# slackhq/nebula

Measured on AMD Instinct MI355X. Metric: GiB/s device-resident AES-256-GCM seal+open, 1300 B pkts, 64 Ki batch, higher is better.
Workload: dtype u8; 1 GPU; C2 AES-256-GCM, 1 tunnel key, 65536 x 1300 B packets, device-resident; packets_per_gpu=65536, payload_bytes_per_pkt=1300, keys=1, cipher=AES-256-GCM, parallelism=1 GPU(s), independent packet shards, no collective

## Files before the change

### nebula_amd/csrc/aes_gcm.hip

```cpp
#include <hip/hip_runtime.h>

#include <atomic>
#include <hip/hip_ext.h>

#include <cstdlib>
#include <cstring>
#include <stdint.h>

#include <type_traits>

#include "../../include/nebula_aead.h"
#include "device_common.hpp"
#include "knobs.hpp"
#include "layout.hpp"
#include "rxwin.hpp"
#include "sched.hpp"
#include "timing.hpp"

#ifdef NEB_ISA_MARKS
#define NEB_MARK(x) asm volatile(";NEBMARK " #x)
#else
#define NEB_MARK(x) ((void)0)
#endif

namespace neb {


struct T0Table {
    uint32_t t[256];
};
constexpr uint8_t kSbox[256] = {
    0x63,0x7c,0x77,0x7b,0xf2,0x6b,0x6f,0xc5,0x30,0x01,0x67,0x2b,0xfe,0xd7,0xab,0x76,
    0xca,0x82,0xc9,0x7d,0xfa,0x59,0x47,0xf0,0xad,0xd4,0xa2,0xaf,0x9c,0xa4,0x72,0xc0,
    0xb7,0xfd,0x93,0x26,0x36,0x3f,0xf7,0xcc,0x34,0xa5,0xe5,0xf1,0x71,0xd8,0x31,0x15,
    0x04,0xc7,0x23,0xc3,0x18,0x96,0x05,0x9a,0x07,0x12,0x80,0xe2,0xeb,0x27,0xb2,0x75,
    0x09,0x83,0x2c,0x1a,0x1b,0x6e,0x5a,0xa0,0x52,0x3b,0xd6,0xb3,0x29,0xe3,0x2f,0x84,
    0x53,0xd1,0x00,0xed,0x20,0xfc,0xb1,0x5b,0x6a,0xcb,0xbe,0x39,0x4a,0x4c,0x58,0xcf,
    0xd0,0xef,0xaa,0xfb,0x43,0x4d,0x33,0x85,0x45,0xf9,0x02,0x7f,0x50,0x3c,0x9f,0xa8,
    0x51,0xa3,0x40,0x8f,0x92,0x9d,0x38,0xf5,0xbc,0xb6,0xda,0x21,0x10,0xff,0xf3,0xd2,
    0xcd,0x0c,0x13,0xec,0x5f,0x97,0x44,0x17,0xc4,0xa7,0x7e,0x3d,0x64,0x5d,0x19,0x73,
    0x60,0x81,0x4f,0xdc,0x22,0x2a,0x90,0x88,0x46,0xee,0xb8,0x14,0xde,0x5e,0x0b,0xdb,
    0xe0,0x32,0x3a,0x0a,0x49,0x06,0x24,0x5c,0xc2,0xd3,0xac,0x62,0x91,0x95,0xe4,0x79,
    0xe7,0xc8,0x37,0x6d,0x8d,0xd5,0x4e,0xa9,0x6c,0x56,0xf4,0xea,0x65,0x7a,0xae,0x08,
    0xba,0x78,0x25,0x2e,0x1c,0xa6,0xb4,0xc6,0xe8,0xdd,0x74,0x1f,0x4b,0xbd,0x8b,0x8a,
    0x70,0x3e,0xb5,0x66,0x48,0x03,0xf6,0x0e,0x61,0x35,0x57,0xb9,0x86,0xc1,0x1d,0x9e,
    0xe1,0xf8,0x98,0x11,0x69,0xd9,0x8e,0x94,0x9b,0x1e,0x87,0xe9,0xce,0x55,0x28,0xdf,
    0x8c,0xa1,0x89,0x0d,0xbf,0xe6,0x42,0x68,0x41,0x99,0x2d,0x0f,0xb0,0x54,0xbb,0x16};

constexpr uint8_t xt(uint8_t a) { return (uint8_t)((a << 1) ^ ((a & 0x80) ? 0x1b : 0)); }
constexpr T0Table make_t0() {
    T0Table r{};
    for (int i = 0; i < 256; i++) {
        uint32_t s = kSbox[i], s2 = xt(kSbox[i]), s3 = s2 ^ s;
        r.t[i] = s2 | (s << 8) | (s << 16) | (s3 << 24);
    }
    return r;
}
__constant__ T0Table c_T0 = make_t0();


__device__ __forceinline__ uint32_t x3(uint32_t a, uint32_t b, uint32_t c) {
    uint32_t r;
    asm("v_bitop3_b32 %0, %1, %2, %3 bitop3:0x96" : "=v"(r) : "v"(a), "v"(b), "v"(c));
    return r;
}
__device__ __forceinline__ uint32_t x3s(uint32_t a, uint32_t b, uint32_t k) {
    uint32_t r;
    asm("v_bitop3_b32 %0, %1, %2, %3 bitop3:0x96" : "=v"(r) : "v"(a), "v"(b), "s"(k));
    return r;
}
__device__ __forceinline__ uint32_t rotl8(uint32_t x) { return __builtin_amdgcn_alignbit(x, x, 24); }
__device__ __forceinline__ uint4 xor4(uint4 a, uint4 b) { return make_uint4(a.x ^ b.x, a.y ^ b.y, a.z ^ b.z, a.w ^ b.w); }
__device__ __forceinline__ uint4 x34(uint4 a, uint4 b, uint4 c) {
    return make_uint4(x3(a.x, b.x, c.x), x3(a.y, b.y, c.y), x3(a.z, b.z, c.z), x3(a.w, b.w, c.w));
}
__device__ __forceinline__ uint4 sel4(bool c, uint4 a, uint4 b) {
    return make_uint4(c ? a.x : b.x, c ? a.y : b.y, c ? a.z : b.z, c ? a.w : b.w);
}
__device__ __forceinline__ uint4 bswap4(uint4 v) { return make_uint4(bswap32(v.x), bswap32(v.y), bswap32(v.z), bswap32(v.w)); }
__device__ __forceinline__ uint4 shfl_xor4(uint4 v, int m) {
    return make_uint4(__shfl_xor(v.x, m), __shfl_xor(v.y, m), __shfl_xor(v.z, m), __shfl_xor(v.w, m));
}
__device__ __forceinline__ uint32_t byte_of(uint32_t w, int k) {
    return k == 0 ? (w & 0xFFu) : (k == 3 ? (w >> 24) : __builtin_amdgcn_ubfe(w, 8 * k, 8));
}

template <class T>
__device__ __forceinline__ T lds_at(const void* base, uint32_t byte_off) {
    return *reinterpret_cast<const T*>(
        __builtin_assume_aligned(reinterpret_cast<const char*>(base) + byte_off, sizeof(T)));
}

__device__ __forceinline__ uint2 ttab_lane_base(uint32_t lane, uint32_t high = 0u) {
    const uint32_t c = lane & 31u, hi = c >> 4;
    return make_uint2((c << 3) | (hi << 2) | high, (c << 3) | ((hi ^ 1u) << 2) | high);
}
__device__ __forceinline__ uint2 ttab_entry(uint32_t i) {
    const uint32_t t = c_T0.t[i >> 5], t2 = __builtin_amdgcn_alignbit(t, t, 16);
    return (i & 16u) ? make_uint2(t2, t) : make_uint2(t, t2);
}

#ifndef NEB_PRIO
#define NEB_PRIO 3
#endif
#ifndef NEB_PRIO_AGE
#define NEB_PRIO_AGE 1
#endif

struct RkRegs {
    const uint32_t* k;
    static constexpr bool kUniform = true;
    static constexpr int kPrioHi = NEB_PRIO, kPrioLo = 0;
    __device__ __forceinline__ uint4 get(int r) const {
        return make_uint4(k[4 * r], k[4 * r + 1], k[4 * r + 2], k[4 * r + 3]);
    }
};
template <int HI, int LO>
struct RkRegsPrio : RkRegs {
    static constexpr int kPrioHi = HI, kPrioLo = LO;
};
struct RkLds {
    const uint4* base;
    static constexpr bool kUniform = false;
    static constexpr int kPrioHi = NEB_PRIO, kPrioLo = 0;
    __device__ __forceinline__ uint4 get(int r) const { return base[r]; }
};

struct TLook {
    const uint2* ttab;
    uint2 lb;
    __device__ __forceinline__ uint32_t t0(uint32_t s, int k) const {
        return lds_at<uint32_t>(ttab, perm(s, lb.x, 0x0C020000u | ((4u + (uint32_t)k) << 8)));
    }
    __device__ __forceinline__ uint32_t t2(uint32_t s, int k) const {
        return lds_at<uint32_t>(ttab, perm(s, lb.y, 0x0C020000u | ((4u + (uint32_t)k) << 8)));
    }
    __device__ __forceinline__ uint32_t t1(uint32_t s, int k) const { return rotl8(t0(s, k)); }
    __device__ __forceinline__ uint32_t t3(uint32_t s, int k) const { return rotl8(t2(s, k)); }
    __device__ __forceinline__ uint32_t t1r(uint32_t s, int k) const { return t0(s, k); }
    __device__ __forceinline__ uint32_t t3r(uint32_t s, int k) const { return t2(s, k); }
    static constexpr bool kFour = false;
};

__device__ __forceinline__ uint32_t ttab4_lane_base(uint32_t lane) {
    const uint32_t c = lane & 31u, hi = c >> 4;
    return ((c << 3) | (hi << 2)) | (1u << 16) | (((c << 3) | ((hi ^ 1u) << 2)) << 24);
}
__device__ __forceinline__ uint2 ttab4_entry(uint32_t i) {
    uint32_t t = c_T0.t[(i >> 5) & 255u];
    if (i & 8192u) t = __builtin_amdgcn_alignbit(t, t, 16);
    const uint32_t t1 = rotl8(t);
    return (i & 16u) ? make_uint2(t1, t) : make_uint2(t, t1);
}
template <uint32_t N, uint32_t THREADS, class F>
__device__ __forceinline__ void fill_ttab(uint2* dst, uint32_t tid, F entry) {
    constexpr uint32_t K = (N + THREADS - 1) / THREADS;
    constexpr bool kWhole = N % THREADS == 0;
    uint2 v[K];
#pragma unroll
    for (uint32_t j = 0; j < K; j++) v[j] = entry((tid + j * THREADS) % N);
#pragma unroll
    for (uint32_t j = 0; j < K; j++)
        if (kWhole || tid + j * THREADS < N) dst[tid + j * THREADS] = v[j];
}
struct TLook4 {
    const uint2* ttab;
    uint32_t lb;
    __device__ __forceinline__ uint32_t at(uint32_t s, int k, uint32_t sel) const {
        return lds_at<uint32_t>(ttab, perm(s, lb, sel | ((4u + (uint32_t)k) << 8)));
    }
    __device__ __forceinline__ uint32_t t0(uint32_t s, int k) const { return at(s, k, 0x0C0C0000u); }
    __device__ __forceinline__ uint32_t t1(uint32_t s, int k) const { return at(s, k, 0x0C0C0003u); }
    __device__ __forceinline__ uint32_t t2(uint32_t s, int k) const { return at(s, k, 0x0C020000u); }
// ... 134 lines not shown
    const uint32_t u1 = c.L.y ^ T.t3(t0, 3);
    const uint32_t u2 = c.L.z ^ T.t2(t0, 2);
    const uint32_t u3 = c.L.w ^ T.t1(t0, 1);
    return aes256_rounds<3>(u0, u1, u2, u3, T, rk);
}


__device__ __forceinline__ uint4 gf_mulx(uint4 v) {
    uint32_t lsb = v.w & 1u;
    uint4 r;
    r.w = shr64(v.z, v.w, 1);
    r.z = shr64(v.y, v.z, 1);
    r.y = shr64(v.x, v.y, 1);
    r.x = (v.x >> 1) ^ (lsb ? 0xE1000000u : 0u);
    return r;
}

__device__ __forceinline__ uint4 gf_reduce(const uint32_t z[8]) {
    const uint32_t l0 = z[4], l1 = z[5], l2 = z[6], l3 = z[7];
    uint32_t t0 = x3(l0, l0 >> 1, l0 >> 2) ^ (l0 >> 7);
    uint32_t t1 = x3(x3(l1, shr64(l0, l1, 1), shr64(l0, l1, 2)), shr64(l0, l1, 7), z[1]);
    uint32_t t2 = x3(x3(l2, shr64(l1, l2, 1), shr64(l1, l2, 2)), shr64(l1, l2, 7), z[2]);
    uint32_t t3 = x3(x3(l3, shr64(l2, l3, 1), shr64(l2, l3, 2)), shr64(l2, l3, 7), z[3]);
    uint32_t o = x3(l3 << 31, l3 << 30, l3 << 25);
    uint32_t of = x3(o, o >> 1, o >> 2) ^ (o >> 7);
    return make_uint4(x3(z[0], t0, of), t1, t2, t3);
}

__device__ __forceinline__ uint4 gf_mul_xpow(uint4 q, uint32_t i) {
    const uint32_t w = i >> 5, b = i & 31u;
    const uint32_t src[4] = {q.x, q.y, q.z, q.w};
    uint32_t y[8], z[8];
#pragma unroll
    for (int k = 0; k < 8; k++) {
        uint32_t v = 0;
#pragma unroll
        for (int j = 0; j < 4; j++) v = (uint32_t)(k - j) == w ? src[j] : v;
        y[k] = v;
    }
    z[0] = y[0] >> b;
#pragma unroll
    for (int k = 1; k < 8; k++) z[k] = shr64(y[k - 1], y[k], b);
    return gf_reduce(z);
}

__device__ __forceinline__ uint4 gf_mul_xpow32(uint4 q, uint32_t b) {
    const uint32_t z[8] = {q.x >> b, shr64(q.x, q.y, b), shr64(q.y, q.z, b), shr64(q.z, q.w, b), shr64(q.w, 0u, b),
                           0u, 0u, 0u};
    return gf_reduce(z);
}

template <int K>
__device__ __forceinline__ uint32_t byte_hi_nibble(uint32_t w) {
    uint32_t r;
    if constexpr (K == 0) {
        r = w & 0xF0u;
    } else {
        asm("v_and_b32_sdwa %0, %1, %2 dst_sel:DWORD dst_unused:UNUSED_PAD src0_sel:BYTE_%c3 src1_sel:DWORD"
            : "=v"(r) : "v"(w), "s"(0xF0u), "i"(K));
    }
    return r;
}

__device__ __forceinline__ uint4 gf_mul_full(uint4 x, uint4 acc, const uint4* ftab) {
    const uint32_t xw[4] = {x.x, x.y, x.z, x.w};
#pragma unroll
    for (int q = 0; q < 4; q++) {
        const uint32_t hi = xw[q];
        const uint32_t lo = xw[q] << 4;
        const uint32_t ah[4] = {byte_hi_nibble<0>(hi), byte_hi_nibble<1>(hi), byte_hi_nibble<2>(hi),
                                byte_hi_nibble<3>(hi)};
        const uint32_t al[4] = {byte_hi_nibble<0>(lo), byte_hi_nibble<1>(lo), byte_hi_nibble<2>(lo),
                                byte_hi_nibble<3>(lo)};
#pragma unroll
        for (int k = 0; k < 4; k++) {
            const uint4 e1 = lds_at<uint4>(ftab, (uint32_t)(8 * q + 6 - 2 * k) * 256u + ah[k]);
            const uint4 e2 = lds_at<uint4>(ftab, (uint32_t)(8 * q + 7 - 2 * k) * 256u + al[k]);
            acc = x34(acc, e1, e2);
        }
    }
    return acc;
}

__device__ __forceinline__ uint4 gf_mul_pos(uint4 x, const uint4* ptab) {
    const uint32_t xw[4] = {x.x, x.y, x.z, x.w};
    uint32_t z[8] = {0, 0, 0, 0, 0, 0, 0, 0};
#pragma unroll
    for (int q = 0; q < 4; q++) {
        const uint32_t hi = xw[q], lo = xw[q] << 4;
        const uint32_t ah[4] = {byte_hi_nibble<0>(hi), byte_hi_nibble<1>(hi), byte_hi_nibble<2>(hi),
                                byte_hi_nibble<3>(hi)};
        const uint32_t al[4] = {byte_hi_nibble<0>(lo), byte_hi_nibble<1>(lo), byte_hi_nibble<2>(lo),
                                byte_hi_nibble<3>(lo)};
#pragma unroll
        for (int k = 0; k < 4; k++) {
            const uint4 e1 = lds_at<uint4>(ptab, (uint32_t)(6 - 2 * k) * 256u + ah[k]);
            const uint4 e2 = lds_at<uint4>(ptab, (uint32_t)(7 - 2 * k) * 256u + al[k]);
            z[q] = x3(z[q], e1.x, e2.x);
            z[q + 1] = x3(z[q + 1], e1.y, e2.y);
            z[q + 2] = x3(z[q + 2], e1.z, e2.z);
            z[q + 3] = x3(z[q + 3], e1.w, e2.w);
        }
    }
    return gf_reduce(z);
}

__device__ __forceinline__ void gf_acc_pos(uint4 x, const uint4* ptab, uint32_t z[8]) {
    const uint32_t xw[4] = {x.x, x.y, x.z, x.w};
#pragma unroll
    for (int q = 0; q < 4; q++) {
        const uint32_t hi = xw[q], lo = xw[q] << 4;
        const uint32_t ah[4] = {byte_hi_nibble<0>(hi), byte_hi_nibble<1>(hi), byte_hi_nibble<2>(hi),
                                byte_hi_nibble<3>(hi)};
        const uint32_t al[4] = {byte_hi_nibble<0>(lo), byte_hi_nibble<1>(lo), byte_hi_nibble<2>(lo),
                                byte_hi_nibble<3>(lo)};
#pragma unroll
        for (int k = 0; k < 4; k++) {
            const uint4 e1 = lds_at<uint4>(ptab, (uint32_t)(6 - 2 * k) * 256u + ah[k]);
            const uint4 e2 = lds_at<uint4>(ptab, (uint32_t)(7 - 2 * k) * 256u + al[k]);
            z[q] = x3(z[q], e1.x, e2.x);
            z[q + 1] = x3(z[q + 1], e1.y, e2.y);
            z[q + 2] = x3(z[q + 2], e1.z, e2.z);
            z[q + 3] = x3(z[q + 3], e1.w, e2.w);
        }
    }
}

__device__ __forceinline__ uint4 gf_mul_pos_off(uint4 x, const void* base, uint32_t off) {
    const uint32_t xw[4] = {x.x, x.y, x.z, x.w};
    uint32_t z[8] = {0, 0, 0, 0, 0, 0, 0, 0};
#pragma unroll
    for (int q = 0; q < 4; q++) {
        const uint32_t hi = xw[q], lo = xw[q] << 4;
        const uint32_t ah[4] = {byte_hi_nibble<0>(hi), byte_hi_nibble<1>(hi), byte_hi_nibble<2>(hi),
                                byte_hi_nibble<3>(hi)};
        const uint32_t al[4] = {byte_hi_nibble<0>(lo), byte_hi_nibble<1>(lo), byte_hi_nibble<2>(lo),
                                byte_hi_nibble<3>(lo)};
#pragma unroll
        for (int k = 0; k < 4; k++) {
            const uint4 e1 = lds_at<uint4>(base, (uint32_t)(6 - 2 * k) * 256u + (ah[k] | off));
            const uint4 e2 = lds_at<uint4>(base, (uint32_t)(7 - 2 * k) * 256u + (al[k] | off));
            z[q] = x3(z[q], e1.x, e2.x);
            z[q + 1] = x3(z[q + 1], e1.y, e2.y);
            z[q + 2] = x3(z[q + 2], e1.z, e2.z);
            z[q + 3] = x3(z[q + 3], e1.w, e2.w);
        }
    }
    return gf_reduce(z);
}

__device__ __forceinline__ uint4 gf_mul_shoup(uint4 x, uint32_t tab, const uint4* base) {
    const uint32_t xw[4] = {x.x, x.y, x.z, x.w};
    uint32_t hi[4], lo[4];
#pragma unroll
    for (int q = 0; q < 4; q++) {
        hi[q] = xw[q] & 0xF0F0F0F0u;
        lo[q] = (xw[q] << 4) & 0xF0F0F0F0u;
    }
    uint32_t z[8] = {0, 0, 0, 0, 0, 0, 0, 0};
#pragma unroll
    for (int r = 0; r < 8; r++) {
        const int k = 3 - (r >> 1);
        uint4 m[4];
#pragma unroll
        for (int q = 0; q < 4; q++) {
            const uint32_t src = (r & 1) ? lo[q] : hi[q];
// ... 120 lines not shown
        const uint64_t abits = (uint64_t)d.aad_len * 8u, cbits = (uint64_t)d.len * 8u;
        X = make_uint4((uint32_t)(abits >> 32), (uint32_t)abits, (uint32_t)(cbits >> 32), (uint32_t)cbits);
        ej0.set(ks);
    }
    return X;
}

template <int CM, class TL, class RK>
__device__ __forceinline__ uint4 gcm_lane_ks(const LaneBlock& b, uint32_t c1, uint32_t c2, const CtrConst& cc,
                                             const TL& T, const RK& rk) {
    if constexpr (CM == 2) return aes256_ctr8_block(cc, b.ctr, T, rk);
    else if constexpr (CM == 1) return aes256_ctr_block(cc, b.ctr, T, rk);
    else return aes256_block(0u, c1, c2, bswap32(b.ctr), T, rk);
}

template <bool OPEN>
__device__ __forceinline__ uint32_t gcm_finish(const neb_desc& d, uint4 S, uint4 ej0, uint32_t lane, uint32_t l,
                                               uint32_t LPP, uint8_t* arena) {
    const uint4 tag = xor4(ej0, bswap4(S));
    uint32_t fail = 0;
    if (l == LPP - 1u) {
        if constexpr (!OPEN) {
            store_block(arena + d.dst_off + d.len, tag, 16);
        } else {
            const uint4 rt = load_block(arena + d.src_off + d.len, 16);
            const uint4 df = xor4(rt, tag);
            fail = (df.x | df.y | df.z | df.w) != 0u;
        }
    }
    if constexpr (OPEN) {
        fail = (uint32_t)__shfl((int)fail, (int)(lane | (LPP - 1u)));
        if (fail) {
            for (uint32_t off = 16u * l; off < d.len; off += 16u * LPP)
                store_block(arena + d.dst_off + off, make_uint4(0, 0, 0, 0), min(16u, d.len - off));
        }
    }
    return fail;
}


constexpr uint32_t kLg = 2;
constexpr uint32_t kLpp = 1u << kLg;
constexpr uint32_t kPpw = 64u / kLpp;
static_assert(kLpp == kFullPow, "the single-key Horner stride is the full table's power");

__device__ __forceinline__ uint4 shfl4(uint4 v, uint32_t src) {
    return make_uint4(__shfl(v.x, (int)src), __shfl(v.y, (int)src), __shfl(v.z, (int)src), __shfl(v.w, (int)src));
}
__device__ __forceinline__ uint4 shfl_down4(uint4 v, uint32_t d) {
    return make_uint4(__shfl_down(v.x, d), __shfl_down(v.y, d), __shfl_down(v.z, d), __shfl_down(v.w, d));
}

struct FinalPermLanes {
    uint32_t src1, src2, off;
};
__device__ __forceinline__ FinalPermLanes final_perm_lanes(uint32_t lane, const uint32_t tab_off[4]) {
    const uint32_t c = (lane >> 2) & 7u, h = lane >> 5;
    const uint32_t g = ((uint32_t)__popc(c) & 1u) + 2u * h;
    const uint32_t i = 4u * (c >> 1) + (lane & 3u);
    const uint32_t l = lane & 3u, q = lane >> 2, m = q >> 2;
    const uint32_t b = (l & 1u) ^ ((uint32_t)__popc(m) & 1u);
    FinalPermLanes f;
    f.src1 = 4u * i + g;
    f.src2 = 32u * (l >> 1) + 4u * (2u * m + b) + (q & 3u);
    f.off = g == 0u ? tab_off[0] : g == 1u ? tab_off[1] : g == 2u ? tab_off[2] : tab_off[3];
    return f;
}
template <int CTRL>
__device__ __forceinline__ uint4 dpp4(uint4 v) {
    return make_uint4((uint32_t)__builtin_amdgcn_mov_dpp((int)v.x, CTRL, 0xF, 0xF, false),
                      (uint32_t)__builtin_amdgcn_mov_dpp((int)v.y, CTRL, 0xF, 0xF, false),
                      (uint32_t)__builtin_amdgcn_mov_dpp((int)v.z, CTRL, 0xF, 0xF, false),
                      (uint32_t)__builtin_amdgcn_mov_dpp((int)v.w, CTRL, 0xF, 0xF, false));
}
template <class MUL>
__device__ __forceinline__ uint4 final_perm(uint4 A, const FinalPermLanes& fp, MUL&& mul) {
    const uint4 a = shfl4(A, fp.src1);
    uint4 v = shfl4(mul(a, fp.off), fp.src2);
    v = xor4(v, dpp4<0xB1>(v));
    return xor4(v, dpp4<0x4E>(v));
}

struct GhFullPerm {
    const uint4* full;
    const void* base;
    FinalPermLanes fp;
    __device__ __forceinline__ uint4 horner(uint4 a, uint32_t) const {
        return gf_mul_full(a, make_uint4(0, 0, 0, 0), full);
    }
    __device__ __forceinline__ uint4 final(uint4 A, uint32_t, uint32_t) const {
        return final_perm(A, fp, [&](uint4 a, uint32_t off) { return gf_mul_pos_off(a, base, off); });
    }
};

template <class OFF>
__device__ __forceinline__ uint4 tree_final(uint4 A, uint32_t lane, uint32_t lg, const uint4* base, OFF&& shoup_off) {
    uint4 V = A;
    for (uint32_t i = 0; i < lg; i++) V = xor4(gf_mul_shoup(V, shoup_off(i), base), shfl_down4(V, 1u << i));
    V = gf_mul_shoup(V, shoup_off(0u), base);
    return shfl4(V, lane & ~((1u << lg) - 1u));
}

#ifndef NEB_TAIL_TREE
#define NEB_TAIL_TREE 0
#endif
struct GhShoup64 {
    const uint4* m16;
    const uint4* shoup;
    const uint4* pos;
    const uint4* hi;
    __device__ __forceinline__ uint4 horner(uint4 a, uint32_t) const { return gf_mul_pos(a, pos); }
    __device__ __forceinline__ uint4 final(uint4 A, uint32_t lane, uint32_t lg) const {
#if NEB_TAIL_TREE
        return tree_final(A, lane, lg, shoup, [](uint32_t i) { return i * 256u; });
#else
        const uint32_t b = lane & 15u, a = (lane >> 4) & 3u;
        uint4 V = gf_mul_shoup(A, (15u - b) * 256u, m16);
        V = xor4(V, shfl_xor4(V, 8));
        V = xor4(V, shfl_xor4(V, 4));
        V = xor4(V, shfl_xor4(V, 2));
        V = xor4(V, shfl_xor4(V, 1));
        const uint4 W = gf_mul_shoup(V, (a < 3u ? 2u - a : 0u) * 256u, hi);
        V = a < 3u ? W : V;
        V = xor4(V, shfl_xor4(V, 16));
        return xor4(V, shfl_xor4(V, 32));
#endif
    }
};

struct GhChunk4 {
    const uint4* shoup;
    const uint4* pos;
    __device__ __forceinline__ uint4 horner(uint4 a, uint32_t) const { return gf_mul_pos(a, pos); }
    __device__ __forceinline__ uint4 final(uint4 A, uint32_t lane, uint32_t) const {
        const uint32_t ln = lane;
        const uint32_t tab_off[4] = {3u * 256u, 2u * 256u, 256u, 0u};
        return final_perm(A, final_perm_lanes(ln, tab_off),
                          [&](uint4 a, uint32_t off) { return gf_mul_shoup(a, off, shoup); });
    }
};
struct GhChunkTail {
    const uint4* shoup;
    const uint4* pos;
    __device__ __forceinline__ uint4 horner(uint4 a, uint32_t) const { return gf_mul_pos(a, pos); }
    __device__ __forceinline__ uint4 final(uint4 A, uint32_t lane, uint32_t lg) const {
        const uint32_t ln = lane;
        const uint32_t tab_off[4] = {3u * 256u, 2u * 256u, 256u, 0u};
        const uint4 Q = final_perm(A, final_perm_lanes(ln, tab_off),
                                   [&](uint4 a, uint32_t off) { return gf_mul_shoup(a, off, shoup); });
        const uint32_t a = (ln >> 2) & ((1u << (lg - 2u)) - 1u);
        const uint4 W = sel4((a & 1u) != 0u, Q, gf_mul_shoup(Q, 3u * 256u, shoup));
        const uint4 P = xor4(W, shfl_xor4(W, 4));
        if (lg == 3u) return P;
        const uint4 U = sel4((a & 2u) != 0u, P, gf_mul_shoup(P, 4u * 256u, shoup));
        return xor4(U, shfl_xor4(U, 8));
    }
};

constexpr uint32_t kCsHdrMask = 0xFFFu;
__device__ __forceinline__ uint32_t le16_sum(uint4 v) {
    return (v.x & 0xFFFFu) + (v.x >> 16) + (v.y & 0xFFFFu) + (v.y >> 16) + (v.z & 0xFFFFu) + (v.z >> 16) +
           (v.w & 0xFFFFu) + (v.w >> 16);
}
__device__ __forceinline__ uint32_t block_byte(uint4 v, uint32_t q) {
    const uint32_t w = q < 4u ? v.x : q < 8u ? v.y : q < 12u ? v.z : v.w;
    return (w >> (8u * (q & 3u))) & 0xFFu;
}
__device__ __forceinline__ uint32_t cs_fold16(uint32_t s) {
    s = (s & 0xFFFFu) + (s >> 16);
    s = (s & 0xFFFFu) + (s >> 16);
    return s;
// ... 126 lines not shown
        auto horner = [&](uint32_t r) -> uint4 { return r == 0 ? make_uint4(0, 0, 0, 0) : gh.horner(A, lg); };
        auto tround = [&](uint32_t r) {
            NEB_MARK(round_begin);
            if (r < sh.R) {
                const LaneBlock b = lane_block(sh, r, l, lg);
                const bool fast = fast_round(b);
                uint4 pre = make_uint4(0, 0, 0, 0);
                if (fast) pre = fast_load(b);
                const uint4 G = horner(r);
                __builtin_amdgcn_sched_barrier(0);
                uint4 ks = make_uint4(0, 0, 0, 0);
                if (__any(b.is_ct || b.is_len)) ks = gcm_lane_ks<CM>(b, c1, c2, cc, T, rk);
                io(b, G, ks, fast, pre);
            }
            NEB_MARK(round_end);
        };
        for (uint32_t r = 0; __any(r < sh.R); r++) tround(r);
    };
#if NEB_ONE_TRACE
    const uint64_t tp0 = __builtin_amdgcn_s_memrealtime();
#endif
    if (__all(sh.m + 1u < 256u)) rounds(std::integral_constant<int, 2>{});
    else if (__all(sh.m + 1u < 65536u)) rounds(std::integral_constant<int, 1>{});
    else rounds(std::integral_constant<int, 0>{});
    if constexpr (CS) {
        for (uint32_t sft = 1; sft < LPP; sft <<= 1) {
            cs_acc += (uint32_t)__shfl_xor((int)cs_acc, (int)sft);
            cs_fk |= (uint32_t)__shfl_xor((int)cs_fk, (int)sft);
        }
    }
#if NEB_ONE_TRACE
    __builtin_amdgcn_s_waitcnt(0);
    const uint64_t tp1 = __builtin_amdgcn_s_memrealtime();
#endif
#ifdef NEB_WAVE_TRACE
    const uint64_t tq2 = phase_now();
    phase_add(1, tq1, tq2);
#endif
    NEB_MARK(rounds_done);
    uint4 V = gh.final(A, lane, lg);
    NEB_MARK(final_done);
#ifdef NEB_WAVE_TRACE
    const uint64_t tq3 = phase_now();
    phase_add(2, tq2, tq3);
#endif
#if NEB_ONE_TRACE
    __builtin_amdgcn_s_waitcnt(0);
    const uint64_t tp2 = __builtin_amdgcn_s_memrealtime();
    if (lane == 0) printf("  rounds %u  final %u (x10 ns, R=%u)\n", (unsigned)(tp1 - tp0), (unsigned)(tp2 - tp1), sh.R);
#endif
    if constexpr (CS) {
        if (run && cs_on && l == LPP - 1u) V = xor4(V, gcm_csum_fix(d, sh.n, sh.na, cs_acc, cs_fk, args.arena, cs_pow));
    }
    if (run && gcm_finish<OPEN>(d, V, ej0.get(), lane, l, LPP, args.arena)) st = NEB_STATUS_AUTH_FAILED;
    if (valid && l == LPP - 1u) args.status[p] = (int32_t)st;
    NEB_MARK(grp_end);
#ifdef NEB_WAVE_TRACE
    phase_add(3, tq3, phase_now());
#endif
}

__device__ __forceinline__ void load_round_keys(const uint32_t* rec, uint32_t rks[60]) {
#pragma unroll
    for (int i = 0; i < 60; i++) rks[i] = __builtin_amdgcn_readfirstlane(rec[kRecRoundKeys + i]);
}

#ifdef NEB_WAVE_TRACE
constexpr uint32_t kWaveTraceSlots = 64, kWaveTraceWaves = 8192, kWaveTraceCap = kWaveTraceSlots * kWaveTraceWaves;
__device__ uint4 g_wtrace[kWaveTraceCap];
__device__ __forceinline__ void wave_trace(uint32_t lane, uint32_t slot, uint32_t a, uint32_t b, uint64_t t0,
                                           uint64_t t1) {
    const uint32_t w = blockIdx.x * (blockDim.x >> 6) + (threadIdx.x >> 6);
    if (lane == 0u && w < kWaveTraceWaves && slot < kWaveTraceSlots)
        g_wtrace[w * kWaveTraceSlots + slot] = make_uint4(a | 0x80000000u, b, (uint32_t)t0, (uint32_t)t1);
}
#endif


constexpr int kSingleWaves = 16;
constexpr int kSingleWpe = 4;
constexpr int kSingleThreads = kSingleWaves * kWave;

struct SingleLds {
    uint4 full[32 * 16];
    uint4 pos1[8 * 16];
    uint2 ttab[2 * 256 * 32];
    uint4 pos23[2][8 * 16];
};
struct SingleLdsCs : SingleLds {
    uint4 pow2[10 * 16];
};

template <bool OPEN, bool CS = false, bool RX = false>
__global__ __launch_bounds__(kSingleThreads, kSingleWpe) void gcm_single_kernel(GcmArgs args) {
    __shared__ std::conditional_t<CS, SingleLdsCs, SingleLds> lds;
    const uint32_t tid = threadIdx.x;
    const uint32_t lane = tid & 63u;
    const uint32_t wave = tid >> 6;
    const uint32_t* srec = args.keys + (size_t)args.key_hint * kKeyRecDwords;
#ifdef NEB_WAVE_TRACE
    const uint64_t tk0 = __builtin_amdgcn_s_memrealtime();
#endif
    static_assert(kSingleThreads >= 512, "one full-table entry per thread");
    uint4 r_full = make_uint4(0, 0, 0, 0), r_h = make_uint4(0, 0, 0, 0), r_p = make_uint4(0, 0, 0, 0);
    if (tid < 512u) r_full = ld_rec4(srec, kRecFull + 4u * tid);
    if (tid < 128u) r_h = ld_rec4(srec, kRecPos1 + 4u * tid);
    if (tid < 256u) r_p = ld_rec4(srec, (tid < 128u ? kRecPos2 : kRecPos3) + 4u * (tid & 127u));
    const TLook4 T{lds.ttab, ttab4_lane_base(lane)};
    fill_ttab<2u * 256u * 32u, kSingleThreads>(lds.ttab, tid, ttab4_entry);
    if (tid < 512u) lds.full[tid] = r_full;
    if (tid < 128u) lds.pos1[tid] = r_h;
    if (tid < 256u) lds.pos23[tid >> 7][tid & 127u] = r_p;

    const uint4* cs_pow = nullptr;
    if constexpr (CS) {
        if (tid < 160u) lds.pow2[tid] = ld_rec4(srec, rec_shoup_pow2(tid >> 4) + 4u * (tid & 15u));
        cs_pow = lds.pow2;
    }
    uint32_t rks[60];
    load_round_keys(srec, rks);
    __syncthreads();
    const RkRegs rk{rks};
    const uint32_t tab_off[4] = {(uint32_t)offsetof(SingleLds, full), (uint32_t)offsetof(SingleLds, pos23[1]),
                                 (uint32_t)offsetof(SingleLds, pos23[0]), (uint32_t)offsetof(SingleLds, pos1)};
    const GhFullPerm gh{lds.full, &lds, final_perm_lanes(lane, tab_off)};

    const bool key_ok = __builtin_amdgcn_readfirstlane(srec[kRecAlg]) == NEB_ALG_AESGCM;
    uint32_t npkt = args.npkt;
    if (args.npkt_dev) npkt = min(npkt, __builtin_amdgcn_readfirstlane(*args.npkt_dev));
    const uint32_t ngroups = (npkt + kPpw - 1u) / kPpw;
    const uint32_t slots = gridDim.x * kSingleWaves;
    uint32_t main_groups = ngroups;
    if (args.tail_slots && ngroups > slots && ngroups % slots)
        main_groups = ngroups / slots * slots;
#ifdef NEB_WAVE_TRACE
    uint32_t trace_k = 1;
    wave_trace(lane, 0, blockIdx.x << 20 | wave << 16, ~0u, tk0, __builtin_amdgcn_s_memrealtime());
#endif
    auto groups = [&](const auto& rkp) {
        for (uint32_t grp = blockIdx.x + wave * gridDim.x; grp < main_groups; grp += slots) {
#ifdef NEB_WAVE_TRACE
            const uint64_t tc0 = __builtin_amdgcn_s_memrealtime();
#endif
            const uint32_t p = grp * kPpw + lane / kLpp;
            gcm_packet_group<OPEN, CS, RX>(args, p, p < npkt, args.key_hint, key_ok, rkp, gh, T, lane, kLg, cs_pow);
#ifdef NEB_WAVE_TRACE
            wave_trace(lane, trace_k++, blockIdx.x << 20 | wave << 16 | 16u << 8 | 2u << 4 | 1u, grp, tc0,
                       __builtin_amdgcn_s_memrealtime());
#endif
        }
    };
#if NEB_PRIO && NEB_PRIO_AGE
    if (__builtin_amdgcn_readfirstlane(wave) >> 3) groups(RkRegsPrio<NEB_PRIO, 1>{rk});
    else groups(rk);
#else
    groups(rk);
#endif
}

constexpr uint32_t kTailLg = 6, kTailPpw = kWave >> kTailLg;
constexpr uint32_t kTailAll = 0xFFFFFFFFu;
constexpr uint32_t kSmallBatch = 6144;
constexpr int kTailWaves = 8;
struct TailLds {
    uint2 ttab[256 * 32];
    uint4 shoup[kTailLg * 16];
    uint4 pos[8 * 16];
    uint4 m16[16 * 16];
    uint4 hi[3 * 16];
};
static_assert(kTailLg == 6, "GhShoup64: 64 lanes per packet");
template <bool OPEN, bool RX = false>
__global__ __launch_bounds__(kTailWaves * kWave) void gcm_single_tail_kernel(GcmArgs args) {
    __shared__ TailLds lds;
    const uint32_t tid = threadIdx.x, lane = tid & 63u, wave = tid >> 6;
    uint32_t npkt = args.npkt;
    if (args.npkt_dev) npkt = min(npkt, __builtin_amdgcn_readfirstlane(*args.npkt_dev));
    const uint32_t ngroups = (npkt + kPpw - 1u) / kPpw, slots = args.tail_slots;
    uint32_t p0 = 0;
    if (slots != kTailAll) {
        if (ngroups <= slots || ngroups % slots == 0u) return;
        p0 = ngroups / slots * slots * kPpw;
    }
    const uint32_t tgroups = (npkt - p0 + kTailPpw - 1u) / kTailPpw;
    if (blockIdx.x * kTailWaves >= tgroups) return;
    const uint32_t* srec = args.keys + (size_t)args.key_hint * kKeyRecDwords;
    fill_ttab<256u * 32u, kTailWaves * kWave>(lds.ttab, tid, ttab_entry);
    if (tid < 16u * kTailLg) {
        const uint32_t j = tid >> 4, v = tid & 15u;
        lds.shoup[tid] = ld_rec4(srec, rec_shoup_pow2(j) + 4u * v);
    }
    if (tid < 128u) lds.pos[tid] = ld_rec4(srec, kRecPos64 + 4u * tid);
    if (tid < 256u) lds.m16[tid] = ld_rec4(srec, kRecShoup + 4u * tid);
    if (tid < 48u) lds.hi[tid] = ld_rec4(srec, (tid < 16u ? kRecShoup + 15u * 64u : tid < 32u ? kRecShoup32 : kRecShoup48) + 4u * (tid & 15u));
    uint32_t rks[60];
    load_round_keys(srec, rks);
    __syncthreads();
    const TLook T{lds.ttab, ttab_lane_base(lane)};
    const GhShoup64 gh{lds.m16, lds.shoup, lds.pos, lds.hi};
    const bool key_ok = __builtin_amdgcn_readfirstlane(srec[kRecAlg]) == NEB_ALG_AESGCM;
    for (uint32_t t = blockIdx.x * kTailWaves + wave; t < tgroups; t += gridDim.x * kTailWaves) {
        const uint32_t p = p0 + kTailPpw * t + (lane >> kTailLg);
        gcm_packet_group<OPEN, false, RX>(args, p, p < npkt, args.key_hint, key_ok, RkRegs{rks}, gh, T, lane, kTailLg);
    }
}

// ... 761 lines not shown
```

Before: 833.4 GiB/s.

## Use 5-bit windowed GHASH multiply tables in single kernel

Replaces the 4-bit nibble table GHASH multiply in the Horner step with a 5-bit window scheme: 26 windows, each doing two 64-bit LDS loads and XOR accumulation. The window tables are built at kernel start by XOR-combining entries of the existing full table. The old full table moves to a new pos4 slot so the final permutation step can still use it. The aim is fewer LDS lookups per GF multiply (52 b64 reads instead of 32 b128 reads), at the cost of more setup work, extra LDS space and volatile loads that may hinder scheduling.

```diff
diff --git a/nebula_amd/csrc/aes_gcm.hip b/nebula_amd/csrc/aes_gcm.hip
--- a/nebula_amd/csrc/aes_gcm.hip
+++ b/nebula_amd/csrc/aes_gcm.hip
@@ -89,6 +89,13 @@
 __device__ __forceinline__ T lds_at(const void* base, uint32_t byte_off) {
     return *reinterpret_cast<const T*>(
         __builtin_assume_aligned(reinterpret_cast<const char*>(base) + byte_off, sizeof(T)));
+}
+
+__device__ __forceinline__ uint2 lds_b64(const void* base, uint32_t byte_off) {
+    typedef uint32_t v2u __attribute__((ext_vector_type(2)));
+    typedef const volatile __attribute__((address_space(3))) v2u* lds_ptr;
+    const v2u v = *(lds_ptr)__builtin_assume_aligned(reinterpret_cast<const char*>(base) + byte_off, 8);
+    return make_uint2(v.x, v.y);
 }
 
 __device__ __forceinline__ uint2 ttab_lane_base(uint32_t lane, uint32_t high = 0u) {
@@ -389,6 +396,35 @@
     return acc;
 }
 
+#ifndef NEB_GHASH5
+#define NEB_GHASH5 1
+#endif
+constexpr int kWin5 = 26;
+__device__ __forceinline__ uint4 gf_mul_full5(uint4 x, uint4 acc, const uint2* f5) {
+    const uint32_t xw[4] = {x.x, x.y, x.z, x.w};
+    uint2 lo[kWin5], hi[kWin5];
+    auto issue = [&](int P) {
+        const int q = (5 * P) >> 5, r = (5 * P) & 31;
+        uint32_t w;
+        if (r > 27 && q < 3) w = __builtin_amdgcn_alignbit(xw[q], xw[q + 1], 56 - r);
+        else w = r <= 24 ? xw[q] >> (24 - r) : xw[q] << (r - 24);
+        const uint32_t a = w & 0xF8u;
+        lo[P] = lds_b64(f5, (uint32_t)(2 * P) * 256u + a);
+        hi[P] = lds_b64(f5, (uint32_t)(2 * P + 1) * 256u + a);
+    };
+    constexpr int kStep = 4;
+#pragma unroll
+    for (int g = 0; g < kWin5; g += kStep) {
+#pragma unroll
+        for (int P = g; P < g + kStep && P < kWin5; P++) issue(P);
+#pragma unroll
+        for (int P = g; P < g + kStep && P < kWin5; P += 2)
+            acc = make_uint4(x3(acc.x, lo[P].x, lo[P + 1].x), x3(acc.y, lo[P].y, lo[P + 1].y),
+                             x3(acc.z, hi[P].x, hi[P + 1].x), x3(acc.w, hi[P].y, hi[P + 1].y));
+    }
+    return acc;
+}
+
 __device__ __forceinline__ uint4 gf_mul_pos(uint4 x, const uint4* ptab) {
     const uint32_t xw[4] = {x.x, x.y, x.z, x.w};
     uint32_t z[8] = {0, 0, 0, 0, 0, 0, 0, 0};
@@ -675,11 +711,19 @@
 }
 
 struct GhFullPerm {
+#if NEB_GHASH5
+    const uint2* full;
+#else
     const uint4* full;
+#endif
     const void* base;
     FinalPermLanes fp;
     __device__ __forceinline__ uint4 horner(uint4 a, uint32_t) const {
+#if NEB_GHASH5
+        return gf_mul_full5(a, make_uint4(0, 0, 0, 0), full);
+#else
         return gf_mul_full(a, make_uint4(0, 0, 0, 0), full);
+#endif
     }
     __device__ __forceinline__ uint4 final(uint4 A, uint32_t, uint32_t) const {
         return final_perm(A, fp, [&](uint4 a, uint32_t off) { return gf_mul_pos_off(a, base, off); });
@@ -972,10 +1016,17 @@
 constexpr int kSingleThreads = kSingleWaves * kWave;
 
 struct SingleLds {
+#if NEB_GHASH5
+    uint2 full[2 * kWin5 * 32];
+#else
     uint4 full[32 * 16];
+#endif
     uint4 pos1[8 * 16];
     uint2 ttab[2 * 256 * 32];
     uint4 pos23[2][8 * 16];
+#if NEB_GHASH5
+    uint4 pos4[8 * 16];
+#endif
 };
 struct SingleLdsCs : SingleLds {
     uint4 pow2[10 * 16];
@@ -991,14 +1042,38 @@
 #ifdef NEB_WAVE_TRACE
     const uint64_t tk0 = __builtin_amdgcn_s_memrealtime();
 #endif
+    uint4 r_full = make_uint4(0, 0, 0, 0), r_h = make_uint4(0, 0, 0, 0), r_p = make_uint4(0, 0, 0, 0);
+#if NEB_GHASH5
+    static_assert(kSingleThreads >= kWin5 * 32, "one window-table entry per thread");
+    const uint32_t f5_p = tid >> 5, f5_v = tid & 31u;
+    if (tid < (uint32_t)kWin5 * 32u) {
+#pragma unroll
+        for (uint32_t j = 0; j < 5u; j++) {
+            const uint32_t b = 5u * f5_p + j, bc = min(b, 127u);
+            const uint4 c = ld_rec4(srec, kRecFull + 4u * ((bc >> 2) * 16u + (8u >> (bc & 3u))));
+            const uint32_t m = (b < 128u && ((f5_v >> (4u - j)) & 1u)) ? ~0u : 0u;
+            r_full = make_uint4(r_full.x ^ (c.x & m), r_full.y ^ (c.y & m), r_full.z ^ (c.z & m), r_full.w ^ (c.w & m));
+        }
+    }
+    if (tid < 128u) r_h = ld_rec4(srec, kRecPos1 + 4u * tid);
+    if (tid < 384u) r_p = ld_rec4(srec, (tid < 128u ? kRecPos2 : tid < 256u ? kRecPos3 : kRecFull) + 4u * (tid & 127u));
+#else
     static_assert(kSingleThreads >= 512, "one full-table entry per thread");
-    uint4 r_full = make_uint4(0, 0, 0, 0), r_h = make_uint4(0, 0, 0, 0), r_p = make_uint4(0, 0, 0, 0);
     if (tid < 512u) r_full = ld_rec4(srec, kRecFull + 4u * tid);
     if (tid < 128u) r_h = ld_rec4(srec, kRecPos1 + 4u * tid);
     if (tid < 256u) r_p = ld_rec4(srec, (tid < 128u ? kRecPos2 : kRecPos3) + 4u * (tid & 127u));
+#endif
     const TLook4 T{lds.ttab, ttab4_lane_base(lane)};
     fill_ttab<2u * 256u * 32u, kSingleThreads>(lds.ttab, tid, ttab4_entry);
+#if NEB_GHASH5
+    if (tid < (uint32_t)kWin5 * 32u) {
+        lds.full[(2u * f5_p) * 32u + f5_v] = make_uint2(r_full.x, r_full.y);
+        lds.full[(2u * f5_p + 1u) * 32u + f5_v] = make_uint2(r_full.z, r_full.w);
+    }
+    if (tid >= 256u && tid < 384u) lds.pos4[tid & 127u] = r_p;
+#else
     if (tid < 512u) lds.full[tid] = r_full;
+#endif
     if (tid < 128u) lds.pos1[tid] = r_h;
     if (tid < 256u) lds.pos23[tid >> 7][tid & 127u] = r_p;
 
@@ -1011,7 +1086,11 @@
     load_round_keys(srec, rks);
     __syncthreads();
     const RkRegs rk{rks};
+#if NEB_GHASH5
+    const uint32_t tab_off[4] = {(uint32_t)offsetof(SingleLds, pos4), (uint32_t)offsetof(SingleLds, pos23[1]),
+#else
     const uint32_t tab_off[4] = {(uint32_t)offsetof(SingleLds, full), (uint32_t)offsetof(SingleLds, pos23[1]),
+#endif
                                  (uint32_t)offsetof(SingleLds, pos23[0]), (uint32_t)offsetof(SingleLds, pos1)};
     const GhFullPerm gh{lds.full, &lds, final_perm_lanes(lane, tab_off)};
 
```

After: 860.7 GiB/s, median of 6. 1.03x the previous value.
